# dselivanov/rsparse

Measured on AMD Instinct MI355X. Metric: als_iterations_per_sec, higher is better.
Workload: dtype f32 (Gram products of rows > 512 / <= 32 non-zeros as 2 x fp16 / 3 x bf16 split terms of the fp32 operands, fp32 accumulate; everything else fp32); 1 GPU; WRMF implicit ALS, CG(3), synthetic 10000000x1000000, 500155883 nnz, rank 128, lambda 0.1; survey_config=3, feedback=implicit, n_items=1000000, nnz=500155883, rank=128, solver=conjugate_gradient, cg_steps=3, parallelism=rows sharded x1, factors replicated

## Files before the change

rsparse_amd/csrc/wrmf_cg_mf.hip:

```cpp
#include <cstdio>
#include <utility>

#pragma clang diagnostic ignored "-Winline-asm"

#include "wrmf_internal.h"
#include "wrmf_device.h"

namespace rsparse_hip {
namespace {
using namespace dev;
constexpr int MF_A0 = 0;
#define MF_TOP "a255"
}
}

#include "wrmf_mf.h"

namespace rsparse_hip {
namespace {

constexpr float kCgTolMf = 1e-10f;
__device__ __forceinline__ void cgm_operands_hi(const float (&x)[16], f16x8& h0, f16x8& h1) {
  float b0[8], b1[8];
#pragma unroll
  for (int e = 0; e < 8; e++) {
    const auto sw2 = __builtin_amdgcn_permlane32_swap(__float_as_uint(x[e]), __float_as_uint(x[8 + e]), false, false);
    b0[e] = __uint_as_float(sw2[0]);
    b1[e] = __uint_as_float(sw2[1]);
  }
  unsigned hh0[4], hh1[4];
#pragma unroll
  for (int q = 0; q < 4; q++) {
    const f32x2 v0 = {b0[2 * q], b0[2 * q + 1]}, v1 = {b1[2 * q], b1[2 * q + 1]};
    hh0[q] = __builtin_bit_cast(unsigned, __builtin_convertvector(v0, f16x2));
    hh1[q] = __builtin_bit_cast(unsigned, __builtin_convertvector(v1, f16x2));
  }
  h0 = mf_pack(hh0[0], hh0[1], hh0[2], hh0[3]);
  h1 = mf_pack(hh1[0], hh1[1], hh1[2], hh1[3]);
}

struct CgmOps {
  f16x8 ah[4], al[4], mh[4];
};
struct CgmProd {
  int T, kind, K, I;
};
constexpr CgmProd cgm_prod(int idx) {
  if (idx < 16) return {mf_tid(idx % 4, 0), idx / 4, 0, idx % 4};
  idx -= 16;
  if (idx < 12) return {mf_tid(1 + idx % 3, 1), idx / 3, 1, 1 + idx % 3};
  idx -= 12;
  const int w = idx % 3, K = w == 2 ? 3 : 2, I = w == 0 ? 2 : 3;
  return {mf_tid(I, K), idx / 3, K, I};
}
template <int T>
__device__ __forceinline__ void cgm_mma16(const f16x8& a, const f16x8& b) {
  asm volatile("v_mfma_f32_32x32x16_f16 a[%c2:%c3], %0, %1, a[%c2:%c3]" ::"v"(a), "v"(b), "i"(MF_A0 + 16 * T), "i"(MF_A0 + 16 * T + 15));
}

template <int NOPS>
struct CgmWave {
  union {
    float ring[3][2048];
    float T[32 * 36];
  };
  int midx[3][64];
  float mval[3][64];
  float gval[3][64];
  unsigned long long maddr[3][64];
  float vec[128];
  float x0[128];
  float rhs[128];
  double loss;
};
template <int NOPS>
struct CgmSmem {
  float4 G[10][64][4];
  CgmWave<NOPS> w[4];
};

template <class RD, class GV, class WV>
__device__ __forceinline__ void cgm_matvec(RD&& rd, GV&& gtile, WV& sw, const int n, const int hf, const int ln,
                                           const float (&pr)[4], float (&out)[4]) {
  wave_sync();
  if (hf == 0) {
#pragma unroll
    for (int I = 0; I < 4; I++) sw.vec[32 * I + n] = pr[I];
  }
  wave_sync();
  float dsum[4] = {0.f, 0.f, 0.f, 0.f};
  mf_sfor<4>([&](auto kt) {
    constexpr int K = decltype(kt)::value;
    float pc[16];
#pragma unroll
    for (int q = 0; q < 4; q++) {
      const float4 t = *reinterpret_cast<const float4*>(&sw.vec[32 * K + 8 * q + 4 * hf]);
      pc[4 * q] = t.x; pc[4 * q + 1] = t.y; pc[4 * q + 2] = t.z; pc[4 * q + 3] = t.w;
    }
    float ts[16];
#pragma unroll
    for (int v = 0; v < 16; v++) ts[v] = 0.f;
    mf_sfor<4 - K>([&](auto st) {
      constexpr int I = K + decltype(st)::value;
      constexpr int T = mf_tid(I, K);
      float g[16];
      gtile(std::integral_constant<int, T>{}, g);
      mf_sfor<16>([&](auto vt) {
        constexpr int v = decltype(vt)::value;
        const float av = rd(std::integral_constant<int, T>{}, std::integral_constant<int, v>{}) + g[v];
        dsum[I] = fmaf(av, pc[v], dsum[I]);
        if constexpr (I > K) ts[v] = fmaf(av, pr[I], ts[v]);
// ... 152 lines not shown
              constexpr int I = K + decltype(st2)::value;
              constexpr int T = mf_tid(I, K);
              if constexpr (T < 6) mf_mma16<10 + T>(mh[K], mh[I]);
              else hi[T - 6] = __builtin_amdgcn_mfma_f32_32x32x16_f16(mh[K], mh[I], hi[T - 6], 0, 0, 0);
            });
          });
        };
        float gj;
        if constexpr (SYM) gj = inl ? __builtin_amdgcn_sqrtf(fmaxf(cvr - 1.f, 0.f) * sw_) : 0.f;
        else gj = f1;
        if constexpr (SYM) {
          cgm_operands_hi(xm0, mh[0], mh[1]);
          cgm_operands_hi(xm1, mh[2], mh[3]);
          __builtin_amdgcn_sched_barrier(0);
          m2_products();
          __builtin_amdgcn_sched_barrier(0);
        } else {
          mf_operands(xm0, bh[0], bl[0], bh[1], bl[1]);
          mf_operands(xm1, bh[2], bl[2], bh[3], bl[3]);
#pragma unroll
          for (int t = 0; t < 4; t++) mh[t] = bh[t];
          __builtin_amdgcn_sched_barrier(0);
          m2_products();
          __builtin_amdgcn_sched_barrier(0);
        }
#pragma unroll
        for (int s2 = 0; s2 < 16; s2++) {
          const float s_a = readlane_f(gj, s2);
          xs0[s2] *= s_a;
          xs1[s2] *= s_a;
        }
        mf_operands(xs0, ah[0], al[0], ah[1], al[1]);
        __builtin_amdgcn_sched_barrier(0);
        mf_operands(xs1, ah[2], al[2], ah[3], al[3]);
        __builtin_amdgcn_sched_barrier(0);
        mf_sfor<3>([&](auto pt) {
          constexpr int pr = decltype(pt)::value;
          mf_sfor<4>([&](auto kt) {
            constexpr int K = decltype(kt)::value;
            mf_sfor<4 - K>([&](auto st2) {
              constexpr int I = K + decltype(st2)::value;
              if constexpr (SYM) mf_mma16<mf_tid(I, K)>(pr == 2 ? al[K] : ah[K], pr == 1 ? al[I] : ah[I]);
              else mf_mma16<mf_tid(I, K)>(pr == 2 ? al[K] : ah[K], pr == 1 ? bl[I] : bh[I]);
            });
          });
        });
      };
      CgmOps OA, OB;
      if constexpr (SYM) {
        const f16x8 z = mf_pack(0u, 0u, 0u, 0u);
#pragma unroll
        for (int t = 0; t < 4; t++) { OA.ah[t] = z; OA.al[t] = z; OA.mh[t] = z; }
      }
      auto mm = [&](auto it, const CgmOps& P) __attribute__((always_inline)) {
        constexpr CgmProd pd = cgm_prod(decltype(it)::value);
        if constexpr (pd.kind == 0) {
          if constexpr (pd.T < 6) cgm_mma16<10 + pd.T>(P.mh[pd.K], P.mh[pd.I]);
          else hi[pd.T - 6] = __builtin_amdgcn_mfma_f32_32x32x16_f16(P.mh[pd.K], P.mh[pd.I], hi[pd.T - 6], 0, 0, 0);
        } else {
          cgm_mma16<pd.T>(pd.kind == 3 ? P.al[pd.K] : P.ah[pd.K], pd.kind == 2 ? P.al[pd.I] : P.ah[pd.I]);
        }
      };
      auto transform = [&](const int c) __attribute__((always_inline)) {
        const int cs = c % 3;
        int l2 = ln;
        asm volatile("" : "+v"(l2));
        const float cvr = sw.mval[cs][l2];
        const int id = sw.midx[cs][l2];
        if constexpr (SYM) csum += p1 + 64 * c + l2 < p2 ? cvr : 0.f;
        wave_sync();
        sw.maddr[cs][l2] = (unsigned long long)(unsigned)id * (k * 4) - (long long)(((l2 & 7) - 4) * 1024);
        if constexpr (SYM) sw.gval[cs][l2] = __builtin_amdgcn_sqrtf(fmaxf(cvr - 1.f, 0.f) * sw_);
        wave_sync();
      };
      auto zero_tail = [&](const int slot, const int ccnt) __attribute__((always_inline)) {
        float* rs = &sw.ring[slot][0];
#pragma unroll 1
        for (int jz = ccnt; jz < 16; jz++) {
          rs[(jz & 7) * 256 + (jz >> 3) * 128 + ln] = 0.f;
          rs[(jz & 7) * 256 + (jz >> 3) * 128 + 64 + ln] = 0.f;
        }
        wave_sync();
      };
      auto step_sym = [&](const int slot, const int cs, auto jt, const CgmOps& P, CgmOps& N, const float4 va0, const float4 vb0, const float2 wc0, const float2 wg0) __attribute__((always_inline)) {
        constexpr int j = decltype(jt)::value;
        const float* rs = &sw.ring[slot][0] + 128 * hfl + 4 * (ln & 31);
        const float2* pc = reinterpret_cast<const float2*>(&sw.mval[cs][16 * j + 8 * hfl]);
        const float2* pg = reinterpret_cast<const float2*>(&sw.gval[cs][16 * j + 8 * hfl]);
        float2 wc[2], wg[2];
        wc[0] = wc0;
        wg[0] = wg0;
        float4 va[2], vb[2];
        va[0] = va0;
        vb[0] = vb0;
        unsigned hm[4][4], hh[4][4], ll[4][4];
        mf_sfor<4>([&](auto qt) {
          constexpr int q = decltype(qt)::value;
          if constexpr (q < 3) {
            va[(q + 1) & 1] = *reinterpret_cast<const float4*>(rs + (2 * q + 2) * 256);
            vb[(q + 1) & 1] = *reinterpret_cast<const float4*>(rs + (2 * q + 3) * 256);
            wc[(q + 1) & 1] = pc[q + 1];
            wg[(q + 1) & 1] = pg[q + 1];
          }
          const float c0 = wc[q & 1].x, c1 = wc[q & 1].y, g0 = wg[q & 1].x, g1 = wg[q & 1].y;
          const float4 xa = va[q & 1], xb = vb[q & 1];
          const float a0s[4] = {xa.x, xa.y, xa.z, xa.w}, a1s[4] = {xb.x, xb.y, xb.z, xb.w};
          mf_sfor<4>([&](auto It) {
            constexpr int I = decltype(It)::value, u = 4 * q + I, m0 = (5 * u) / 2, m1 = (5 * (u + 1)) / 2;
            const float a0 = a0s[I], a1 = a1s[I];
            ua[I] = fmaf(c1, a1, fmaf(c0, a0, ua[I]));
            const float t0 = a0 * sx, t1 = a1 * sx;
            {
              const f32x2 tv = {t0, t1};
              hm[I][q] = __builtin_bit_cast(unsigned, __builtin_convertvector(tv, f16x2));
            }
            mm(std::integral_constant<int, m0>{}, P);
            __builtin_amdgcn_sched_barrier(0);
            {
              const f32x2 yv = {t0 * g0, t1 * g1};
              const unsigned hv = __builtin_bit_cast(unsigned, __builtin_convertvector(yv, f16x2));
              float r0, r1;
              asm("v_fma_mix_f32 %0, %1, %2, -%3 op_sel_hi:[0,0,1]" : "=v"(r0) : "v"(t0), "v"(g0), "v"(hv));
              asm("v_fma_mix_f32 %0, %1, %2, -%3 op_sel:[0,0,1] op_sel_hi:[0,0,1]" : "=v"(r1) : "v"(t1), "v"(g1), "v"(hv));
              const f32x2 rv = {r0, r1};
              hh[I][q] = hv;
              ll[I][q] = __builtin_bit_cast(unsigned, __builtin_convertvector(rv, f16x2));
            }
            mm(std::integral_constant<int, m0 + 1>{}, P);
            if constexpr (m1 - m0 == 3) {
              __builtin_amdgcn_sched_barrier(0);
              mm(std::integral_constant<int, m0 + 2>{}, P);
            }
            __builtin_amdgcn_sched_barrier(0);
          });
        });
#pragma unroll
        for (int I = 0; I < 4; I++) {
          N.mh[I] = mf_pack(hm[I][0], hm[I][1], hm[I][2], hm[I][3]);
          N.ah[I] = mf_pack(hh[I][0], hh[I][1], hh[I][2], hh[I][3]);
          N.al[I] = mf_pack(ll[I][0], ll[I][1], ll[I][2], ll[I][3]);
        }
      };
      wave_sync();
      request_meta(0);
      request_meta(1);
      asm volatile("s_waitcnt vmcnt(0)" ::: "memory");
      transform(0);
      request(0, 0);
      request(1, 1);
      const int tail_st = ((p2 - p1) & 15) ? nsteps - 1 : -1;
      int slot = 0;
      for (int c = 0; 4 * c < nsteps; c++) {
        bool done = false;
        mf_sfor<4>([&](auto jt) {
          constexpr int j = decltype(jt)::value;
          const int st = 4 * c + j;
          if (done || st >= nsteps) { done = true; return; }
          const int slot2 = slot == 0 ? 2 : slot - 1;
          float4 fva, fvb;
          float2 fwc, fwg;
          auto first_reads = [&](const int sl, const int cs, const int jj) __attribute__((always_inline)) {
            const float* rs = &sw.ring[sl][0] + 128 * hfl + 4 * (ln & 31);
            fva = *reinterpret_cast<const float4*>(rs);
            fvb = *reinterpret_cast<const float4*>(rs + 256);
            fwc = *reinterpret_cast<const float2*>(&sw.mval[cs][16 * jj + 8 * hfl]);
            fwg = *reinterpret_cast<const float2*>(&sw.gval[cs][16 * jj + 8 * hfl]);
          };
          if constexpr (j == 1) transform(c + 1);
          const bool more = st + 2 < nsteps;
          if (more) {
            if constexpr (j == 1) asm volatile("s_waitcnt vmcnt(10)" ::: "memory");
            else asm volatile("s_waitcnt vmcnt(8)" ::: "memory");
            if constexpr (SYM) first_reads(slot, c % 3, j);
            request(st + 2, slot2);
            if constexpr (j == 0) request_meta(c + 2);
          } else {
            asm volatile("s_waitcnt vmcnt(0)" ::: "memory");
            if constexpr (SYM) {
              if (st == tail_st) zero_tail(slot, (p2 - p1) & 15);
              first_reads(slot, c % 3, j);
            }
          }
          if constexpr (SYM) {
            __builtin_amdgcn_sched_barrier(0);
            if constexpr (j & 1) step_sym(slot, c % 3, jt, OB, OA, fva, fvb, fwc, fwg);
            else step_sym(slot, c % 3, jt, OA, OB, fva, fvb, fwc, fwg);
          } else {
            const float cvr = sw.mval[c % 3][16 * j + (ln & 15)];
            const float* rs = &sw.ring[slot][0];
            float xs0[16], xs1[16];
#pragma unroll
            for (int s2 = 0; s2 < 16; s2++) {
              xs0[s2] = rs[(s2 & 7) * 256 + (s2 >> 3) * 128 + 4 * (ln & 31) + hfl];
              xs1[s2] = rs[(s2 & 7) * 256 + (s2 >> 3) * 128 + 4 * (ln & 31) + 2 + hfl];
            }
            __builtin_amdgcn_sched_barrier(0);
            consume(st, cvr, xs0, xs1);
            __builtin_amdgcn_sched_barrier(0);
          }
          slot = slot == 2 ? 0 : slot + 1;
        });
        if (done) break;
      }
      if constexpr (SYM) {
        if (nsteps & 1) mf_sfor<40>([&](auto it) { mm(it, OB); });
        else mf_sfor<40>([&](auto it) { mm(it, OA); });
#pragma unroll
        for (int I = 0; I < 4; I++) {
          const unsigned du = __float_as_uint(ua[I]);
          const auto sw2 = __builtin_amdgcn_permlane32_swap(du, du, false, false);
          ua[I] = __uint_as_float(sw2[0]) + __uint_as_float(sw2[1]);
        }
      }
      wave_sync();
    }
    ln = lane;
    asm volatile("" : "+v"(ln));
    const int n = ln & 31, hf = ln >> 5;
    const float un_m1 = (un1 * un1) * (SYM ? unw : unw), un_m2 = un1 * un1;
    MF_DRAIN();
    mf_sfor<160>([&](auto rt) {
      constexpr int R = decltype(rt)::value;
      mf_wr<R>(mf_rd<R>() * un_m1);
    });
    mf_sfor<96>([&](auto rt) {
      constexpr int R = 160 + decltype(rt)::value;
      mf_wr<R>(mf_rd<R>() * un_m2);
    });
    {
      float um = un_m2;
      asm volatile("" : "+v"(um));
#pragma unroll
      for (int t = 0; t < 4; t++)
#pragma unroll
        for (int e = 0; e < 16; e++) hi[t][e] *= um;
    }
    float b[4], x[4];
    if constexpr (SYM) {
#pragma unroll
      for (int I = 0; I < 4; I++) {
        b[I] = ua[I];
        x[I] = sw.x0[4 * n + I];
      }
    } else {
      wave_sync();
      sw.rhs[ln] = u0;
      sw.rhs[64 + ln] = u1;
      wave_sync();
#pragma unroll
      for (int I = 0; I < 4; I++) {
        b[I] = sw.rhs[32 * I + n];
        x[I] = sw.x0[4 * n + I];
      }
    }
    auto rd_m1 = [&](auto tt, auto vt) { return mf_rd<16 * decltype(tt)::value + decltype(vt)::value>(); };
    auto g_tile = [&](auto tt, float (&g)[16]) {
      constexpr int T = decltype(tt)::value;
#pragma unroll
      for (int q = 0; q < 4; q++) {
        const float4 t = sm.G[T][ln][q];
        g[4 * q] = t.x; g[4 * q + 1] = t.y; g[4 * q + 2] = t.z; g[4 * q + 3] = t.w;
      }
    };
    float r[4], p[4], ap[4];
    cgm_matvec(rd_m1, g_tile, sw, n, hf, ln, x, ap);
#pragma unroll
    for (int I = 0; I < 4; I++) { r[I] = b[I] - ap[I]; p[I] = r[I]; }
    double rsold = (double)cgm_dot(r, r, hf);
    for (int stp = 0; stp < a.cg_steps; stp++) {
      cgm_matvec(rd_m1, g_tile, sw, n, hf, ln, p, ap);
      const float alpha = (float)(rsold / (double)cgm_dot(p, ap, hf));
#pragma unroll
      for (int I = 0; I < 4; I++) { x[I] = fmaf(alpha, p[I], x[I]); r[I] = fmaf(-alpha, ap[I], r[I]); }
// ... 92 lines not shown
```

rsparse_amd/csrc/wrmf_kernels.hip:

```cpp
#include "wrmf_internal.h"
#include "wrmf_device.h"

namespace rsparse_hip {
namespace {

using namespace dev;

constexpr float kCgTol = 1e-10f;

template <int KP, int T, int W, bool IMPLICIT>
struct CgSmem {
  static constexpr int LDT = Geo<KP>::LDT;
  static constexpr size_t gram_floats = IMPLICIT ? (size_t)KP * KP : 0;
  static constexpr size_t tile_floats = (size_t)W * T * LDT;
  static constexpr size_t vec_floats = (size_t)W * KP;
  static constexpr size_t red_floats = (size_t)2 * W * KP + 2 * W;
  static constexpr size_t short_bytes = (gram_floats + tile_floats + vec_floats) * 4 + 16;
  static constexpr size_t long_bytes = (gram_floats + tile_floats + vec_floats + red_floats) * 4 + 16;
};

template <int KP, int W>
__device__ __forceinline__ void load_gram_lds(float* sG, const float* __restrict__ G, int k, int tid) {
  for (int e = tid; e < KP * KP; e += W * 64) {
    const int r = e / KP, c = e % KP;
// ... 251 lines not shown
          for (int u = 0; u < EPL; u++) out[u] = fmaf(mode == 0 ? -lam_use : lam_use, v[u], out[u]);
        } else if (gb && mode == 0) {
#pragma unroll
          for (int u = 0; u < EPL; u++) out[u] += (active && e0 + u < k) ? a.rhs_init[e0 + u] : 0.f;
        }
      }
      buf ^= 1;
    };

    float dummy = 0.f;
    sweep(x, 0, r, dummy);
    float rs = 0.f;
#pragma unroll
    for (int u = 0; u < EPL; u++) { p[u] = r[u]; rs = fmaf(r[u], r[u], rs); }
    float rsold = wave_sum(rs);
    for (int it = 0; it < a.cg_steps; ++it) {
      sweep(p, 1, ap, dummy);
      float pap = 0.f;
#pragma unroll
      for (int u = 0; u < EPL; u++) pap = fmaf(p[u], ap[u], pap);
      pap = wave_sum(pap);
      const float alpha = (float)((double)rsold / (double)pap);
      rs = 0.f;
#pragma unroll
      for (int u = 0; u < EPL; u++) {
        x[u] = fmaf(alpha, p[u], x[u]);
        r[u] = fmaf(-alpha, ap[u], r[u]);
        rs = fmaf(r[u], r[u], rs);
      }
      const float rsnew = wave_sum(rs);
      if (rsnew < kCgTol) break;
      const float beta = (float)((double)rsnew / (double)rsold);
#pragma unroll
      for (int u = 0; u < EPL; u++) p[u] = fmaf(p[u], beta, r[u]);
      rsold = rsnew;
    }
    float rl = 0.f;
    sweep(x, 2, ap, rl);
    float xx = 0.f;
#pragma unroll
    for (int u = 0; u < EPL; u++) xx = fmaf(x[u], x[u], xx);
    xx = wave_sum(xx);
    if (wv == 0) {
      wloss += IMPLICIT ? (double)rl + a.lambda_loss * (double)xx : (double)(rl + lam_use * xx);
#pragma unroll
      for (int u = 0; u < EPL; u++)
        if (active && e0 + u < k) yrow[e0 + u] = x[u];
    }
  }
  if (tid == 0) a.loss_partials[loss_slot0 + blockIdx.x] = wloss;
}

typedef float f32x16 __attribute__((ext_vector_type(16)));

template <int KP>
__global__ __launch_bounds__(256, 2) void gramian_partial_kernel(const float* __restrict__ X, int k, int64_t n,
                                                              float* __restrict__ partials,
                                                              unsigned* __restrict__ absmax_bits) {
  constexpr int NT = KP / 32, U = 4;
  const int lane = threadIdx.x & 63;
  const int64_t gw = (int64_t)blockIdx.x * 4 + (threadIdx.x >> 6), nw = (int64_t)gridDim.x * 4;
  const int col = lane & 31, half = lane >> 5;
  f32x16 acc[NT][NT];
#pragma unroll
  for (int i = 0; i < NT; i++)
#pragma unroll
    for (int j = 0; j < NT; j++)
#pragma unroll
      for (int e = 0; e < 16; e++) acc[i][j][e] = 0.f;

  float amax = 0.f;
  auto fetch = [&](const int64_t n0, float (&dst)[U][NT]) {
#pragma unroll
    for (int u = 0; u < U; u++) {
      const int64_t ent = n0 + 2 * u + half;
      const int64_t er = ent < n ? ent : n - 1;
#pragma unroll
      for (int mt = 0; mt < NT; mt++) dst[u][mt] = X[er * k + min(mt * 32 + col, k - 1)];
    }
  };
  auto take = [&](const int64_t n0, const float (&src)[U][NT], float (&dst)[U][NT]) {
#pragma unroll
    for (int u = 0; u < U; u++) {
      const bool in = n0 + 2 * u + half < n;
#pragma unroll
      for (int mt = 0; mt < NT; mt++) dst[u][mt] = src[u][mt] * ((in && mt * 32 + col < k) ? 1.f : 0.f);
    }
  };
  float av[U][NT], nx[U][NT];
  const int64_t stride = nw * 2 * U;
  int64_t n0 = gw * 2 * U;
  if (n0 < n) {
    fetch(n0, nx);
    take(n0, nx, av);
  }
  for (; n0 < n; n0 += stride) {
    const bool more = n0 + stride < n;
    if (more) fetch(n0 + stride, nx);
#pragma unroll
    for (int u = 0; u < U; u++)
#pragma unroll
      for (int mt = 0; mt < NT; mt++) amax = fmaxf(amax, fabsf(av[u][mt]));
#pragma unroll
    for (int u = 0; u < U; u++)
#pragma unroll
      for (int mt = 0; mt < NT; mt++)
#pragma unroll
        for (int nt = 0; nt <= mt; nt++)
          acc[mt][nt] = __builtin_amdgcn_mfma_f32_32x32x2f32(av[u][mt], av[u][nt], acc[mt][nt], 0, 0, 0);
    if (more) take(n0 + stride, nx, av);
  }
  if (absmax_bits) {
#pragma unroll
    for (int off = 32; off > 0; off >>= 1) amax = fmaxf(amax, __shfl_xor(amax, off));
    if (lane == 0) atomicMax(absmax_bits, __float_as_uint(amax < 3.0e38f ? amax : 3.0e38f));
  }
  float* out = partials + (size_t)gw * KP * KP;
#pragma unroll
  for (int mt = 0; mt < NT; mt++)
#pragma unroll
    for (int nt = 0; nt <= mt; nt++)
#pragma unroll
      for (int e = 0; e < 16; e++) {
        const int rr = mt * 32 + (e & 3) + 8 * (e >> 2) + 4 * half;
        out[(size_t)rr * KP + nt * 32 + col] = acc[mt][nt][e];
      }
}

__global__ void gramian_reduce_kernel(const float* __restrict__ partials, int nparts, int KP, int k, float ridge,
                                      float* __restrict__ G, double* __restrict__ diag) {
  const int e = blockIdx.x * blockDim.x + threadIdx.x;
  if (e >= k * k) return;
  const int aa = e / k, bb = e % k;
  const int ta = aa / 32, tb = bb / 32;
  const int rr = ta >= tb ? aa : bb, cc = ta >= tb ? bb : aa;
  double s = 0.0;
  const float* src = partials + (size_t)rr * KP + cc;
  for (int w = 0; w < nparts; w++) s += (double)src[(size_t)w * KP * KP];
  G[(size_t)bb * k + aa] = (float)s + (aa == bb ? ridge : 0.f);
  if (aa == bb) diag[aa] = s;
}

__global__ void trace_kernel(const double* __restrict__ diag, int k, double* __restrict__ out) {
  if (threadIdx.x == 0 && blockIdx.x == 0) {
    double s = 0.0;
    for (int i = 0; i < k; i++) s += diag[i];
    *out = s;
  }
}

__global__ __launch_bounds__(256) void weighted_sumsq_kernel(const float* __restrict__ X, int k, int64_t n,
                                                             const float* __restrict__ w, double* __restrict__ partials) {
  __shared__ double sh[4];
  const int64_t total = n * k;
  double s = 0.0;
  for (int64_t e = (int64_t)blockIdx.x * 256 + threadIdx.x; e < total; e += (int64_t)gridDim.x * 256) {
    const float v = X[e];
    const float wj = w ? w[e / k] : 1.f;
    s += (double)(v * v * wj);
  }
  for (int m = 32; m >= 1; m >>= 1) s += __shfl_xor(s, m);
  if ((threadIdx.x & 63) == 0) sh[threadIdx.x >> 6] = s;
  __syncthreads();
  if (threadIdx.x == 0) partials[blockIdx.x] = (sh[0] + sh[1]) + (sh[2] + sh[3]);
}

__global__ __launch_bounds__(256) void sum_partials_kernel(const double* __restrict__ partials, size_t n,
                                                           double* __restrict__ out) {
  __shared__ double sh[4];
  double s = 0.0;
  for (size_t e = threadIdx.x; e < n; e += 256) s += partials[e];
  for (int m = 32; m >= 1; m >>= 1) s += __shfl_xor(s, m);
  if ((threadIdx.x & 63) == 0) sh[threadIdx.x >> 6] = s;
  __syncthreads();
  if (threadIdx.x == 0) *out = (sh[0] + sh[1]) + (sh[2] + sh[3]);
}

__global__ __launch_bounds__(256) void sum_partials_stage_kernel(const double* __restrict__ partials, size_t n,
                                                                 double* __restrict__ tail) {
  __shared__ double sh[4];
  const size_t per = (n + gridDim.x - 1) / gridDim.x, lo = (size_t)blockIdx.x * per, hi = lo + per < n ? lo + per : n;
  double s = 0.0;
  for (size_t e = lo + threadIdx.x; e < hi; e += 256) s += partials[e];
  for (int m = 32; m >= 1; m >>= 1) s += __shfl_xor(s, m);
  if ((threadIdx.x & 63) == 0) sh[threadIdx.x >> 6] = s;
  __syncthreads();
  if (threadIdx.x == 0) tail[blockIdx.x] = (sh[0] + sh[1]) + (sh[2] + sh[3]);
}

__global__ void f64_to_f32_kernel(const double* __restrict__ in, float* __restrict__ out, size_t n) {
  for (size_t e = (size_t)blockIdx.x * blockDim.x + threadIdx.x; e < n; e += (size_t)gridDim.x * blockDim.x)
    out[e] = (float)in[e];
}
__global__ void f32_to_f64_kernel(const float* __restrict__ in, double* __restrict__ out, size_t n) {
  for (size_t e = (size_t)blockIdx.x * blockDim.x + threadIdx.x; e < n; e += (size_t)gridDim.x * blockDim.x)
    out[e] = (double)in[e];
}

template <typename K>
hipError_t set_lds(K kernel, size_t bytes) {
// ... 25 lines not shown
    if ((err = hipGetLastError()) != hipSuccess) return err;
  }
  if (ev && (err = hipEventRecord(ev[2], s)) != hipSuccess) return err;
  return hipSuccess;
}

}

int padded_rank(int k) {
  if (k <= 0) return 0;
  if (k <= 32) return 32;
  if (k <= 64) return 64;
  if (k <= 128) return 128;
  return 0;
}

size_t cg_loss_slots(int n_cols, int n_long) {
  const size_t grid_s = ((size_t)n_cols + kRowsPerWGShort - 1) / kRowsPerWGShort;
  const size_t grid_l = ((size_t)n_long + kRowsPerWGLong - 1) / kRowsPerWGLong;
  return grid_s * kWavesPerWG + grid_l;
}

size_t chol_loss_slots(int n_cols) {
  return (size_t)(n_cols < kCholMaxGrid ? (n_cols > 0 ? n_cols : 1) : kCholMaxGrid);
}

hipError_t launch_als_cg(const AlsArgs& a, bool implicit, hipStream_t s, hipEvent_t* ev) {
  const int KP = padded_rank(a.k);
  const bool vec = (a.k % 4 == 0) && ((reinterpret_cast<uintptr_t>(a.X) & 15) == 0);
#define RSP_DISPATCH(KPV)                                                             \
  if (KP == KPV) {                                                                    \
    if (implicit) return vec ? launch_cg_t<KPV, true, true>(a, s, ev) : launch_cg_t<KPV, true, false>(a, s, ev); \
    return vec ? launch_cg_t<KPV, false, true>(a, s, ev) : launch_cg_t<KPV, false, false>(a, s, ev);             \
  }
  RSP_DISPATCH(32)
  RSP_DISPATCH(64)
  RSP_DISPATCH(128)
#undef RSP_DISPATCH
  return hipErrorInvalidValue;
}

hipError_t launch_sum_partials(const double* partials, size_t n, double* out, hipStream_t s, double* tail) {
  if (tail && n > 16384) {
    hipLaunchKernelGGL(sum_partials_stage_kernel, dim3(kSumStageBlocks), dim3(256), 0, s, partials, n, tail);
    hipError_t err = hipGetLastError();
    if (err != hipSuccess) return err;
    hipLaunchKernelGGL(sum_partials_kernel, dim3(1), dim3(256), 0, s, tail, (size_t)kSumStageBlocks, out);
    return hipGetLastError();
  }
  hipLaunchKernelGGL(sum_partials_kernel, dim3(1), dim3(256), 0, s, partials, n, out);
  return hipGetLastError();
}

static int gramian_waves(int64_t n) {
  int64_t w = (n + 63) / 64;
  if (w < 1) w = 1;
  if (w > 1024) w = 1024;
  return (int)((w + 3) / 4 * 4);
}

size_t gramian_scratch_floats(int k, int64_t n) {
  const int KP = padded_rank(k);
  return (size_t)gramian_waves(n) * KP * KP + 2 * 128  + 16;
}

hipError_t launch_gramian(const float* X, int k, int64_t n, float ridge, float* XtX, double* sumsq,
                          float* scratch, hipStream_t s, hipEvent_t* ev, unsigned* absmax_bits) {
  const int KP = padded_rank(k);
  if (!KP) return hipErrorInvalidValue;
  const int waves = gramian_waves(n);
  float* partials = scratch;
  double* diag = reinterpret_cast<double*>(scratch + (((size_t)waves * KP * KP + 1) & ~(size_t)1));
  const int grid = waves / 4;
  if (ev) (void)hipEventRecord(ev[0], s);
  prof_note(ev, KP == 32 ? reinterpret_cast<const void*>(gramian_partial_kernel<32>)
                         : (KP == 64 ? reinterpret_cast<const void*>(gramian_partial_kernel<64>)
                                     : reinterpret_cast<const void*>(gramian_partial_kernel<128>)));
  prof_note(ev ? ev + 1 : nullptr, reinterpret_cast<const void*>(gramian_reduce_kernel));
  if (KP == 32) hipLaunchKernelGGL(gramian_partial_kernel<32>, dim3(grid), dim3(256), 0, s, X, k, n, partials, absmax_bits);
  else if (KP == 64) hipLaunchKernelGGL(gramian_partial_kernel<64>, dim3(grid), dim3(256), 0, s, X, k, n, partials, absmax_bits);
  else hipLaunchKernelGGL(gramian_partial_kernel<128>, dim3(grid), dim3(256), 0, s, X, k, n, partials, absmax_bits);
  hipError_t err = hipGetLastError();
  if (err != hipSuccess) return err;
  if (ev) (void)hipEventRecord(ev[1], s);
  hipLaunchKernelGGL(gramian_reduce_kernel, dim3((k * k + 255) / 256), dim3(256), 0, s, partials, waves, KP, k,
                     ridge, XtX, diag);
  if ((err = hipGetLastError()) != hipSuccess) return err;
  if (sumsq) {
    hipLaunchKernelGGL(trace_kernel, dim3(1), dim3(64), 0, s, diag, k, sumsq);
    err = hipGetLastError();
  }
  if (ev) (void)hipEventRecord(ev[2], s);
  return err;
}

hipError_t launch_weighted_sumsq(const float* X, int k, int64_t n, const float* w, double* out, double* scratch,
                                 hipStream_t s) {
  int64_t blocks = (n * k + 256 * 16 - 1) / (256 * 16);
  if (blocks < 1) blocks = 1;
  if (blocks > 1024) blocks = 1024;
  hipLaunchKernelGGL(weighted_sumsq_kernel, dim3((int)blocks), dim3(256), 0, s, X, k, n, w, scratch);
  hipError_t err = hipGetLastError();
  if (err != hipSuccess) return err;
  return launch_sum_partials(scratch, (size_t)blocks, out, s);
}

hipError_t launch_f64_to_f32(const double* in, float* out, size_t n, hipStream_t s) {
  if (!n) return hipSuccess;
  size_t blocks = (n + 1023) / 1024;
  if (blocks > 4096) blocks = 4096;
  hipLaunchKernelGGL(f64_to_f32_kernel, dim3((int)blocks), dim3(256), 0, s, in, out, n);
  return hipGetLastError();
}
hipError_t launch_f32_to_f64(const float* in, double* out, size_t n, hipStream_t s) {
  if (!n) return hipSuccess;
  size_t blocks = (n + 1023) / 1024;
  if (blocks > 4096) blocks = 4096;
  hipLaunchKernelGGL(f32_to_f64_kernel, dim3((int)blocks), dim3(256), 0, s, in, out, n);
  return hipGetLastError();
}

}
```

Measured before the change: 8.506 iterations/s.

## Merge symmetric cross terms of split-fp16 Gram into doubled products

Reorders the split-precision product schedule for the symmetric Gram case. On diagonal tiles the hi*lo and lo*hi cross terms are merged into one MFMA against a doubled low operand, which cuts the per-row products from 40 to 36. Afterwards each diagonal 32x32 accumulator tile is symmetrized through LDS (averaged with its transpose) to restore exact symmetry. This adds VALU doubling work, LDS round trips in the epilogue, and a small precision risk from doubling the fp16 low part.

```diff
diff --git a/rsparse_amd/csrc/wrmf_cg_mf.hip b/rsparse_amd/csrc/wrmf_cg_mf.hip
--- a/rsparse_amd/csrc/wrmf_cg_mf.hip
+++ b/rsparse_amd/csrc/wrmf_cg_mf.hip
@@ -45,18 +45,38 @@
 struct CgmProd {
   int T, kind, K, I;
 };
+constexpr int kCgmProds = 36;
 constexpr CgmProd cgm_prod(int idx) {
-  if (idx < 16) return {mf_tid(idx % 4, 0), idx / 4, 0, idx % 4};
-  idx -= 16;
-  if (idx < 12) return {mf_tid(1 + idx % 3, 1), idx / 3, 1, 1 + idx % 3};
-  idx -= 12;
-  const int w = idx % 3, K = w == 2 ? 3 : 2, I = w == 0 ? 2 : 3;
-  return {mf_tid(I, K), idx / 3, K, I};
-}
+  constexpr int tab[kCgmProds][3] = {
+      {0, 0, 0}, {0, 0, 1}, {0, 0, 2}, {0, 0, 3}, {1, 0, 0}, {1, 0, 1}, {1, 0, 2}, {1, 0, 3}, {2, 0, 0}, {2, 0, 1}, {2, 0, 2}, {2, 0, 3},
+      {3, 0, 1}, {3, 0, 2}, {3, 0, 3},
+      {0, 1, 1}, {0, 1, 2}, {2, 1, 1}, {0, 1, 3}, {1, 1, 1}, {1, 1, 2}, {1, 1, 3}, {2, 1, 2}, {2, 1, 3}, {3, 1, 2}, {3, 1, 3},
+      {2, 2, 2}, {0, 2, 2}, {0, 2, 3}, {0, 3, 3}, {1, 2, 3}, {1, 2, 2}, {2, 2, 3}, {1, 3, 3}, {3, 2, 3}, {2, 3, 3}};
+  return {mf_tid(tab[idx][2], tab[idx][1]), tab[idx][0], tab[idx][1], tab[idx][2]};
+}
+constexpr bool cgm_doubled(int idx) { return cgm_prod(idx).kind == 2 && cgm_prod(idx).I == cgm_prod(idx).K; }
+constexpr int cgm_doubled_in(int m0, int m1) {
+  for (int i = m0; i < m1; i++)
+    if (cgm_doubled(i)) return i;
+  return -1;
+}
+constexpr bool cgm_table_ok() {
+  int seen[10][4] = {};
+  for (int i = 0; i < kCgmProds; i++) {
+    const CgmProd p = cgm_prod(i);
+    if (p.I < p.K || p.I > 3 || p.kind > 3 || (p.kind == 3 && p.I == p.K)) return false;
+    if (seen[p.T][p.kind]++) return false;
+    if (i && cgm_prod(i - 1).T == p.T && (cgm_prod(i - 1).kind == 0) == (p.kind == 0)) return false;
+    if (cgm_doubled(i) != (i == 8 || i == 17 || i == 26 || i == 35)) return false;
+  }
+  return true;
+}
+static_assert(cgm_table_ok(), "cgm_prod");
 template <int T>
 __device__ __forceinline__ void cgm_mma16(const f16x8& a, const f16x8& b) {
   asm volatile("v_mfma_f32_32x32x16_f16 a[%c2:%c3], %0, %1, a[%c2:%c3]" ::"v"(a), "v"(b), "i"(MF_A0 + 16 * T), "i"(MF_A0 + 16 * T + 15));
 }
+__device__ __forceinline__ f16x8 cgm_twice(const f16x8& l) { return l + l; }
 
 template <int NOPS>
 struct CgmWave {
@@ -315,11 +335,13 @@
 #pragma unroll
         for (int t = 0; t < 4; t++) { OA.ah[t] = z; OA.al[t] = z; OA.mh[t] = z; }
       }
-      auto mm = [&](auto it, const CgmOps& P) __attribute__((always_inline)) {
+      auto mm = [&](auto it, const CgmOps& P, const f16x8& b2) __attribute__((always_inline)) {
         constexpr CgmProd pd = cgm_prod(decltype(it)::value);
         if constexpr (pd.kind == 0) {
           if constexpr (pd.T < 6) cgm_mma16<10 + pd.T>(P.mh[pd.K], P.mh[pd.I]);
           else hi[pd.T - 6] = __builtin_amdgcn_mfma_f32_32x32x16_f16(P.mh[pd.K], P.mh[pd.I], hi[pd.T - 6], 0, 0, 0);
+        } else if constexpr (cgm_doubled(decltype(it)::value)) {
+          cgm_mma16<pd.T>(P.ah[pd.K], b2);
         } else {
           cgm_mma16<pd.T>(pd.kind == 3 ? P.al[pd.K] : P.ah[pd.K], pd.kind == 2 ? P.al[pd.I] : P.ah[pd.I]);
         }
@@ -369,15 +391,22 @@
           const float4 xa = va[q & 1], xb = vb[q & 1];
           const float a0s[4] = {xa.x, xa.y, xa.z, xa.w}, a1s[4] = {xb.x, xb.y, xb.z, xb.w};
           mf_sfor<4>([&](auto It) {
-            constexpr int I = decltype(It)::value, u = 4 * q + I, m0 = (5 * u) / 2, m1 = (5 * (u + 1)) / 2;
+            constexpr int I = decltype(It)::value, u = 4 * q + I, m0 = (9 * u) / 4, m1 = (9 * (u + 1)) / 4;
             const float a0 = a0s[I], a1 = a1s[I];
+            constexpr int md = cgm_doubled_in(m0, m1);
+            f16x8 b2 = P.al[0];
+            if constexpr (md >= 0) b2 = cgm_twice(P.al[cgm_prod(md >= 0 ? md : 0).I]);
             ua[I] = fmaf(c1, a1, fmaf(c0, a0, ua[I]));
             const float t0 = a0 * sx, t1 = a1 * sx;
             {
               const f32x2 tv = {t0, t1};
               hm[I][q] = __builtin_bit_cast(unsigned, __builtin_convertvector(tv, f16x2));
             }
-            mm(std::integral_constant<int, m0>{}, P);
+            if constexpr (md >= 0) {
+              static_assert(md < 0 || md == m0 + 2, "the copy's distance to its matrix instruction");
+              asm volatile("" : "+v"(b2));
+            }
+            mm(std::integral_constant<int, m0>{}, P, b2);
             __builtin_amdgcn_sched_barrier(0);
             {
               const f32x2 yv = {t0 * g0, t1 * g1};
@@ -389,10 +418,10 @@
               hh[I][q] = hv;
               ll[I][q] = __builtin_bit_cast(unsigned, __builtin_convertvector(rv, f16x2));
             }
-            mm(std::integral_constant<int, m0 + 1>{}, P);
+            mm(std::integral_constant<int, m0 + 1>{}, P, b2);
             if constexpr (m1 - m0 == 3) {
               __builtin_amdgcn_sched_barrier(0);
-              mm(std::integral_constant<int, m0 + 2>{}, P);
+              mm(std::integral_constant<int, m0 + 2>{}, P, b2);
             }
             __builtin_amdgcn_sched_barrier(0);
           });
@@ -466,8 +495,15 @@
         if (done) break;
       }
       if constexpr (SYM) {
-        if (nsteps & 1) mf_sfor<40>([&](auto it) { mm(it, OB); });
-        else mf_sfor<40>([&](auto it) { mm(it, OA); });
+        auto last_mm = [&](const CgmOps& P) __attribute__((always_inline)) {
+          f16x8 b2[4];
+#pragma unroll
+          for (int I = 0; I < 4; I++) b2[I] = cgm_twice(P.al[I]);
+          asm volatile("s_nop 1" : "+v"(b2[0]), "+v"(b2[1]), "+v"(b2[2]), "+v"(b2[3]));
+          mf_sfor<kCgmProds>([&](auto it) { mm(it, P, b2[cgm_prod(decltype(it)::value).I]); });
+        };
+        if (nsteps & 1) last_mm(OB);
+        else last_mm(OA);
 #pragma unroll
         for (int I = 0; I < 4; I++) {
           const unsigned du = __float_as_uint(ua[I]);
@@ -482,6 +518,23 @@
     const int n = ln & 31, hf = ln >> 5;
     const float un_m1 = (un1 * un1) * (SYM ? unw : unw), un_m2 = un1 * un1;
     MF_DRAIN();
+    if constexpr (SYM) {
+      mf_sfor<4>([&](auto dt) {
+        constexpr int R0 = 16 * mf_tid(decltype(dt)::value, decltype(dt)::value);
+        float d[16];
+        mf_sfor<16>([&](auto vt) { d[decltype(vt)::value] = mf_rd<R0 + decltype(vt)::value>(); });
+        wave_sync();
+#pragma unroll
+        for (int q = 0; q < 4; q++)
+          *reinterpret_cast<float4*>(&sw.T[n * 36 + 8 * q + 4 * hf]) = make_float4(d[4 * q], d[4 * q + 1], d[4 * q + 2], d[4 * q + 3]);
+        wave_sync();
+        mf_sfor<16>([&](auto vt) {
+          constexpr int v = decltype(vt)::value;
+          mf_wr<R0 + v>(0.5f * (d[v] + sw.T[(8 * (v >> 2) + 4 * hf + (v & 3)) * 36 + n]));
+        });
+      });
+      wave_sync();
+    }
     mf_sfor<160>([&](auto rt) {
       constexpr int R = decltype(rt)::value;
       mf_wr<R>(mf_rd<R>() * un_m1);
```

After: 8.547 iterations/s (median of 6 runs). No clear change (+0.5%).

## Rewrite Gramian with 3-term bf16 split MFMA, LDS partial sums, fused reduce

Applied to the files above, without the earlier changes.

Replaces the fp32 32x32x2 MFMA Gramian with a bf16 32x32x16 MFMA path. Each fp32 operand is split into three bf16 terms and six cross-products are accumulated. Rows are fetched with buffer loads in a prefetching chain, and an exponent lift guards tiny inputs. Per-wave accumulators are flushed into LDS and summed per workgroup, which cuts the partial count from up to 1024 waves to 256 workgroups. The reduce kernel now reads float4 partials, writes both triangles of G, and folds the trace into a last-block-done atomic, which drops a kernel launch. Risks include precision loss from the bf16 split, heavy register and LDS pressure at occupancy 1, and a changed lane-to-column mapping that must match the reduce indexing.

```diff
diff --git a/rsparse_amd/csrc/wrmf_kernels.hip b/rsparse_amd/csrc/wrmf_kernels.hip
--- a/rsparse_amd/csrc/wrmf_kernels.hip
+++ b/rsparse_amd/csrc/wrmf_kernels.hip
@@ -327,100 +327,247 @@
 }
 
 typedef float f32x16 __attribute__((ext_vector_type(16)));
-
-template <int KP>
-__global__ __launch_bounds__(256, 2) void gramian_partial_kernel(const float* __restrict__ X, int k, int64_t n,
+typedef float f32x2g __attribute__((ext_vector_type(2)));
+typedef __bf16 bf16x2g __attribute__((ext_vector_type(2)));
+typedef __bf16 bf16x8g __attribute__((ext_vector_type(8)));
+typedef unsigned u32x4g __attribute__((ext_vector_type(4)));
+
+constexpr int kGramTrip = 16;
+constexpr int kGramMaxWGs = 256;
+constexpr int kGramChain = 4;
+
+__host__ __device__ constexpr int gram_tiles(int KP) { return (KP / 32) * (KP / 32 + 1) / 2; }
+__host__ __device__ constexpr int gram_partial_floats(int KP) { return gram_tiles(KP) * 16 * 64; }
+
+__device__ __forceinline__ unsigned gram_split_stage(f32x2g& r, bool last) {
+  const bf16x2g hb = __builtin_convertvector(r, bf16x2g);
+  const unsigned pk = __builtin_bit_cast(unsigned, hb);
+  if (!last) {
+    const f32x2g hi = {__uint_as_float(pk << 16), __uint_as_float(pk & 0xffff0000u)};
+    r -= hi;
+  }
+  return pk;
+}
+__device__ __forceinline__ f32x16 gram_mfma(const u32x4g a, const u32x4g b, const f32x16 c) {
+  return __builtin_amdgcn_mfma_f32_32x32x16_bf16(__builtin_bit_cast(bf16x8g, a), __builtin_bit_cast(bf16x8g, b), c, 0, 0,
+                                                 0);
+}
+
+template <int KP, bool VEC>
+__global__ __launch_bounds__(256, 1) void gramian_partial_kernel(const float* __restrict__ X, int k, int64_t n,
                                                               float* __restrict__ partials,
-                                                              unsigned* __restrict__ absmax_bits) {
-  constexpr int NT = KP / 32, U = 4;
-  const int lane = threadIdx.x & 63;
-  const int64_t gw = (int64_t)blockIdx.x * 4 + (threadIdx.x >> 6), nw = (int64_t)gridDim.x * 4;
-  const int col = lane & 31, half = lane >> 5;
+                                                              unsigned* __restrict__ absmax_bits,
+                                                              unsigned* __restrict__ done_count) {
+  constexpr int NT = KP / 32, E = kGramTrip / 2;
+  typedef float rowv __attribute__((ext_vector_type(NT)));
+  constexpr int TILES = gram_tiles(KP);
+  extern __shared__ __attribute__((aligned(16))) float gsum[];
+  const int lane = threadIdx.x & 63, wv = rfl(threadIdx.x >> 6);
+  const int64_t gw = (int64_t)blockIdx.x * 4 + wv, nw = (int64_t)gridDim.x * 4;
+  const int row = lane & 31, half = lane >> 5;
+  if (done_count && blockIdx.x == 0 && threadIdx.x == 0) *done_count = 0;
   f32x16 acc[NT][NT];
-#pragma unroll
-  for (int i = 0; i < NT; i++)
-#pragma unroll
-    for (int j = 0; j < NT; j++)
-#pragma unroll
-      for (int e = 0; e < 16; e++) acc[i][j][e] = 0.f;
+  float4* mysum = reinterpret_cast<float4*>(gsum + wv * TILES * 1024) + lane;
+
+  bool cin[NT];
+#pragma unroll
+  for (int I = 0; I < NT; I++) cin[I] = NT * row + I < k;
 
   float amax = 0.f;
-  auto fetch = [&](const int64_t n0, float (&dst)[U][NT]) {
-#pragma unroll
-    for (int u = 0; u < U; u++) {
-      const int64_t ent = n0 + 2 * u + half;
-      const int64_t er = ent < n ? ent : n - 1;
-#pragma unroll
-      for (int mt = 0; mt < NT; mt++) dst[u][mt] = X[er * k + min(mt * 32 + col, k - 1)];
+  float rawA[E][NT], rawB[E][NT];
+  unsigned voff[VEC ? 1 : NT];
+#pragma unroll
+  for (int I = 0; I < (VEC ? 1 : NT); I++)
+    voff[I] = (unsigned)(E * half * k + (VEC ? min(NT * row, k - NT) : min(NT * row + I, k - 1))) * 4u;
+  auto fetch = [&](float (&raw)[E][NT], const int64_t n0) {
+    const int rem = (int)max((int64_t)0, min((int64_t)kGramTrip, n - n0));
+#pragma unroll
+    for (int j = 0; j < E; j++) {
+      const __amdgpu_buffer_rsrc_t rs = __builtin_amdgcn_make_buffer_rsrc(
+          const_cast<float*>(X + (n0 + j) * k), 0, j < rem ? (rem - j) * k * 4 : 0, 0x00020000);
+      if constexpr (VEC && NT == 4) {
+        const u32x4g v = __builtin_amdgcn_raw_buffer_load_b128(rs, voff[0], 0, 0);
+#pragma unroll
+        for (int I = 0; I < NT; I++) raw[j][I] = __uint_as_float(v[I]);
+      } else if constexpr (VEC && NT == 2) {
+        typedef unsigned u32x2g __attribute__((ext_vector_type(2)));
+        const u32x2g v = __builtin_amdgcn_raw_buffer_load_b64(rs, voff[0], 0, 0);
+        raw[j][0] = __uint_as_float(v[0]);
+        raw[j][1] = __uint_as_float(v[1]);
+      } else {
+#pragma unroll
+        for (int I = 0; I < NT; I++)
+          raw[j][I] = __uint_as_float(__builtin_amdgcn_raw_buffer_load_b32(rs, voff[VEC ? 0 : I], 0, 0));
+      }
     }
   };
-  auto take = [&](const int64_t n0, const float (&src)[U][NT], float (&dst)[U][NT]) {
-#pragma unroll
-    for (int u = 0; u < U; u++) {
-      const bool in = n0 + 2 * u + half < n;
-#pragma unroll
-      for (int mt = 0; mt < NT; mt++) dst[u][mt] = src[u][mt] * ((in && mt * 32 + col < k) ? 1.f : 0.f);
-    }
+  const int64_t stride = nw * kGramTrip;
+  int lift = -1;
+  float lift_f = 1.f;
+  auto trip = [&](float (&raw)[E][NT], const int64_t n_next) {
+    __builtin_amdgcn_sched_barrier(0);
+    u32x4g term[NT][3];
+#pragma unroll
+    for (int j = 0; j < E; j += 2)
+#pragma unroll
+      for (int I = 0; I < NT; I++) {
+        f32x2g r = {cin[I] ? raw[j][I] * lift_f : 0.f, cin[I] ? raw[j + 1][I] * lift_f : 0.f};
+        amax = fmaxf(amax, fmaxf(fabsf(r.x), fabsf(r.y)));
+        term[I][0][j / 2] = gram_split_stage(r, false);
+        term[I][1][j / 2] = gram_split_stage(r, false);
+        term[I][2][j / 2] = gram_split_stage(r, true);
+      }
+    __builtin_amdgcn_sched_barrier(0);
+    fetch(raw, n_next);
+    __builtin_amdgcn_sched_barrier(0);
+#pragma unroll
+    for (int mt = 0; mt < NT; mt++)
+#pragma unroll
+      for (int nt = 0; nt <= mt; nt++) {
+        f32x16 c = acc[mt][nt];
+        c = gram_mfma(term[mt][0], term[nt][0], c);
+        c = gram_mfma(term[mt][0], term[nt][1], c);
+        c = gram_mfma(term[mt][1], term[nt][0], c);
+        c = gram_mfma(term[mt][0], term[nt][2], c);
+        c = gram_mfma(term[mt][2], term[nt][0], c);
+        c = gram_mfma(term[mt][1], term[nt][1], c);
+        acc[mt][nt] = c;
+      }
   };
-  float av[U][NT], nx[U][NT];
-  const int64_t stride = nw * 2 * U;
-  int64_t n0 = gw * 2 * U;
-  if (n0 < n) {
-    fetch(n0, nx);
-    take(n0, nx, av);
-  }
-  for (; n0 < n; n0 += stride) {
-    const bool more = n0 + stride < n;
-    if (more) fetch(n0 + stride, nx);
-#pragma unroll
-    for (int u = 0; u < U; u++)
-#pragma unroll
-      for (int mt = 0; mt < NT; mt++) amax = fmaxf(amax, fabsf(av[u][mt]));
-#pragma unroll
-    for (int u = 0; u < U; u++)
+  for (;;) {
+#pragma unroll
+    for (int i = 0; i < NT; i++)
+#pragma unroll
+      for (int j = 0; j < NT; j++)
+#pragma unroll
+        for (int e = 0; e < 16; e++) acc[i][j][e] = 0.f;
+    for (int i = 0; i < TILES * 4; i++) mysum[i * 64] = make_float4(0.f, 0.f, 0.f, 0.f);
+    amax = 0.f;
+    int64_t n0 = gw * kGramTrip;
+    fetch(rawA, n0);
+    fetch(rawB, n0 + stride);
+    if (lift < 0) {
+      float m = 0.f;
+#pragma unroll
+      for (int j = 0; j < E; j++)
+#pragma unroll
+        for (int I = 0; I < NT; I++) m = fmaxf(m, cin[I] ? fabsf(rawA[j][I]) : 0.f);
+#pragma unroll
+      for (int off = 32; off > 0; off >>= 1) m = fmaxf(m, __shfl_xor(m, off));
+      lift = (m > 0.f && m < 0x1p-40f) ? rfl(-40 - ilogbf(m)) : 0;
+      lift_f = ldexpf(1.f, lift);
+    }
+    for (; n0 < n; n0 += kGramChain * stride) {
+      trip(rawA, n0 + 2 * stride);
+      if (n0 + stride < n) trip(rawB, n0 + 3 * stride);
+      if (n0 + 2 * stride < n) trip(rawA, n0 + 4 * stride);
+      if (n0 + 3 * stride < n) trip(rawB, n0 + 5 * stride);
+      int t = 0;
 #pragma unroll
       for (int mt = 0; mt < NT; mt++)
 #pragma unroll
-        for (int nt = 0; nt <= mt; nt++)
-          acc[mt][nt] = __builtin_amdgcn_mfma_f32_32x32x2f32(av[u][mt], av[u][nt], acc[mt][nt], 0, 0, 0);
-    if (more) take(n0 + stride, nx, av);
+        for (int nt = 0; nt <= mt; nt++, t++)
+#pragma unroll
+          for (int e = 0; e < 16; e += 4) {
+            float4 v = mysum[(t * 4 + e / 4) * 64];
+            v.x += acc[mt][nt][e];
+            v.y += acc[mt][nt][e + 1];
+            v.z += acc[mt][nt][e + 2];
+            v.w += acc[mt][nt][e + 3];
+            mysum[(t * 4 + e / 4) * 64] = v;
+            acc[mt][nt][e] = acc[mt][nt][e + 1] = acc[mt][nt][e + 2] = acc[mt][nt][e + 3] = 0.f;
+          }
+    }
+#pragma unroll
+    for (int off = 32; off > 0; off >>= 1) amax = fmaxf(amax, __shfl_xor(amax, off));
+    if (lift == 0 || amax <= 0x1p30f) break;
+    lift = 0;
+    lift_f = 1.f;
+  }
+  if (lift) {
+    amax = ldexpf(amax, -lift);
+    for (int i = 0; i < TILES * 4; i++) {
+      float4 v = mysum[i * 64];
+      v.x = ldexpf(v.x, -2 * lift);
+      v.y = ldexpf(v.y, -2 * lift);
+      v.z = ldexpf(v.z, -2 * lift);
+      v.w = ldexpf(v.w, -2 * lift);
+      mysum[i * 64] = v;
+    }
   }
   if (absmax_bits) {
-#pragma unroll
-    for (int off = 32; off > 0; off >>= 1) amax = fmaxf(amax, __shfl_xor(amax, off));
     if (lane == 0) atomicMax(absmax_bits, __float_as_uint(amax < 3.0e38f ? amax : 3.0e38f));
   }
-  float* out = partials + (size_t)gw * KP * KP;
-#pragma unroll
-  for (int mt = 0; mt < NT; mt++)
-#pragma unroll
-    for (int nt = 0; nt <= mt; nt++)
-#pragma unroll
-      for (int e = 0; e < 16; e++) {
-        const int rr = mt * 32 + (e & 3) + 8 * (e >> 2) + 4 * half;
-        out[(size_t)rr * KP + nt * 32 + col] = acc[mt][nt][e];
-      }
-}
-
-__global__ void gramian_reduce_kernel(const float* __restrict__ partials, int nparts, int KP, int k, float ridge,
-                                      float* __restrict__ G, double* __restrict__ diag) {
-  const int e = blockIdx.x * blockDim.x + threadIdx.x;
-  if (e >= k * k) return;
-  const int aa = e / k, bb = e % k;
-  const int ta = aa / 32, tb = bb / 32;
-  const int rr = ta >= tb ? aa : bb, cc = ta >= tb ? bb : aa;
-  double s = 0.0;
-  const float* src = partials + (size_t)rr * KP + cc;
-  for (int w = 0; w < nparts; w++) s += (double)src[(size_t)w * KP * KP];
-  G[(size_t)bb * k + aa] = (float)s + (aa == bb ? ridge : 0.f);
-  if (aa == bb) diag[aa] = s;
-}
-
-__global__ void trace_kernel(const double* __restrict__ diag, int k, double* __restrict__ out) {
-  if (threadIdx.x == 0 && blockIdx.x == 0) {
-    double s = 0.0;
-    for (int i = 0; i < k; i++) s += diag[i];
-    *out = s;
+  __syncthreads();
+  float* out = partials + (size_t)blockIdx.x * gram_partial_floats(KP);
+  for (int t = 0; t < TILES; t++) {
+    const int i = (t * 4 + wv) * 256 + lane * 4;
+    const float4 a0 = *reinterpret_cast<const float4*>(gsum + i), a1 = *reinterpret_cast<const float4*>(gsum + TILES * 1024 + i);
+    const float4 a2 = *reinterpret_cast<const float4*>(gsum + 2 * TILES * 1024 + i);
+    const float4 a3 = *reinterpret_cast<const float4*>(gsum + 3 * TILES * 1024 + i);
+    const float r[4] = {(a0.x + a1.x) + (a2.x + a3.x), (a0.y + a1.y) + (a2.y + a3.y), (a0.z + a1.z) + (a2.z + a3.z),
+                        (a0.w + a1.w) + (a2.w + a3.w)};
+#pragma unroll
+    for (int q = 0; q < 4; q++) out[(t * 16 + 4 * wv + q) * 64 + lane] = r[q];
+  }
+}
+
+__global__ __launch_bounds__(256) void gramian_reduce_kernel(const float* __restrict__ partials, int nparts, int KP, int k,
+                                                             float ridge, float* __restrict__ G, double* diag,
+                                                             unsigned* done_count, double* __restrict__ sumsq) {
+  __shared__ double sh[16][64];
+  __shared__ bool last;
+  const int tid = threadIdx.x, q = tid & 15, g = tid >> 4;
+  const int NT = KP / 32;
+  const size_t pf = (size_t)gram_partial_floats(KP);
+  const float* src = partials + (size_t)blockIdx.x * 64 + 4 * q;
+  double s0 = 0.0, s1 = 0.0, s2 = 0.0, s3 = 0.0;
+#pragma unroll 4
+  for (int p = g; p < nparts; p += 16) {
+    const float4 v = *reinterpret_cast<const float4*>(src + p * pf);
+    s0 += (double)v.x;
+    s1 += (double)v.y;
+    s2 += (double)v.z;
+    s3 += (double)v.w;
+  }
+  sh[g][4 * q + 0] = s0;
+  sh[g][4 * q + 1] = s1;
+  sh[g][4 * q + 2] = s2;
+  sh[g][4 * q + 3] = s3;
+  __syncthreads();
+  for (int h = 8; h >= 1; h >>= 1) {
+    if (g < h)
+#pragma unroll
+      for (int u = 0; u < 4; u++) sh[g][4 * q + u] += sh[g + h][4 * q + u];
+    __syncthreads();
+  }
+  if (tid < 64) {
+    const int t = blockIdx.x / 16, e = blockIdx.x % 16;
+    int mt = 0;
+    while ((mt + 1) * (mt + 2) / 2 <= t) mt++;
+    const int nt = t - mt * (mt + 1) / 2;
+    const int i = (e & 3) + 8 * (e >> 2) + 4 * (tid >> 5), j = tid & 31;
+    const int a = NT * i + mt, b = NT * j + nt;
+    const double s = sh[0][tid];
+    if (a < k && b < k && (mt != nt || i >= j)) {
+      const float v = (float)s + (a == b ? ridge : 0.f);
+      G[(size_t)a * k + b] = v;
+      G[(size_t)b * k + a] = v;
+      if (a == b && sumsq) diag[a] = s;
+    }
+  }
+  if (!sumsq) return;
+  __threadfence();
+  __syncthreads();
+  if (tid == 0) last = atomicAdd(done_count, 1u) == gridDim.x - 1;
+  __syncthreads();
+  if (last && tid < 64) {
+    __threadfence();
+    double v = 0.0;
+    if (tid < k) v = __hip_atomic_load(diag + tid, __ATOMIC_RELAXED, __HIP_MEMORY_SCOPE_AGENT);
+    if (tid + 64 < k) v += __hip_atomic_load(diag + tid + 64, __ATOMIC_RELAXED, __HIP_MEMORY_SCOPE_AGENT);
+    for (int m = 32; m >= 1; m >>= 1) v += __shfl_xor(v, m);
+    if (tid == 0) *sumsq = v;
   }
 }
 
@@ -552,44 +699,50 @@
   return hipGetLastError();
 }
 
-static int gramian_waves(int64_t n) {
-  int64_t w = (n + 63) / 64;
+static int gramian_wgs(int64_t n) {
+  int64_t w = (n + 4 * kGramTrip - 1) / (4 * kGramTrip);
   if (w < 1) w = 1;
-  if (w > 1024) w = 1024;
-  return (int)((w + 3) / 4 * 4);
+  if (w > kGramMaxWGs) w = kGramMaxWGs;
+  return (int)w;
 }
 
 size_t gramian_scratch_floats(int k, int64_t n) {
   const int KP = padded_rank(k);
-  return (size_t)gramian_waves(n) * KP * KP + 2 * 128  + 16;
+  return (size_t)gramian_wgs(n) * gram_partial_floats(KP) + 2 * 128  + 16 ;
+}
+
+template <int KP>
+static hipError_t launch_gramian_partial(bool vec, int grid, hipStream_t s, hipEvent_t* ev, const float* X, int k, int64_t n,
+                                   float* partials, unsigned* absmax_bits, unsigned* done_count) {
+  auto kern = vec ? gramian_partial_kernel<KP, true> : gramian_partial_kernel<KP, false>;
+  const size_t lds = (size_t)4 * gram_partial_floats(KP) * sizeof(float);
+  hipError_t err = set_lds(kern, lds);
+  if (err != hipSuccess) return err;
+  prof_note(ev, reinterpret_cast<const void*>(kern));
+  hipLaunchKernelGGL(kern, dim3(grid), dim3(256), lds, s, X, k, n, partials, absmax_bits, done_count);
+  return hipGetLastError();
 }
 
 hipError_t launch_gramian(const float* X, int k, int64_t n, float ridge, float* XtX, double* sumsq,
                           float* scratch, hipStream_t s, hipEvent_t* ev, unsigned* absmax_bits) {
   const int KP = padded_rank(k);
   if (!KP) return hipErrorInvalidValue;
-  const int waves = gramian_waves(n);
+  const int grid = gramian_wgs(n), NT = KP / 32;
   float* partials = scratch;
-  double* diag = reinterpret_cast<double*>(scratch + (((size_t)waves * KP * KP + 1) & ~(size_t)1));
-  const int grid = waves / 4;
+  double* diag = reinterpret_cast<double*>(scratch + (size_t)grid * gram_partial_floats(KP));
+  unsigned* done_count = reinterpret_cast<unsigned*>(diag + 128);
+  const bool vec = (k % NT == 0) && ((reinterpret_cast<uintptr_t>(X) & (size_t)(4 * NT - 1)) == 0);
   if (ev) (void)hipEventRecord(ev[0], s);
-  prof_note(ev, KP == 32 ? reinterpret_cast<const void*>(gramian_partial_kernel<32>)
-                         : (KP == 64 ? reinterpret_cast<const void*>(gramian_partial_kernel<64>)
-                                     : reinterpret_cast<const void*>(gramian_partial_kernel<128>)));
+  hipError_t err;
+  if (KP == 32) err = launch_gramian_partial<32>(vec, grid, s, ev, X, k, n, partials, absmax_bits, done_count);
+  else if (KP == 64) err = launch_gramian_partial<64>(vec, grid, s, ev, X, k, n, partials, absmax_bits, done_count);
+  else err = launch_gramian_partial<128>(vec, grid, s, ev, X, k, n, partials, absmax_bits, done_count);
+  if (err != hipSuccess) return err;
   prof_note(ev ? ev + 1 : nullptr, reinterpret_cast<const void*>(gramian_reduce_kernel));
-  if (KP == 32) hipLaunchKernelGGL(gramian_partial_kernel<32>, dim3(grid), dim3(256), 0, s, X, k, n, partials, absmax_bits);
-  else if (KP == 64) hipLaunchKernelGGL(gramian_partial_kernel<64>, dim3(grid), dim3(256), 0, s, X, k, n, partials, absmax_bits);
-  else hipLaunchKernelGGL(gramian_partial_kernel<128>, dim3(grid), dim3(256), 0, s, X, k, n, partials, absmax_bits);
-  hipError_t err = hipGetLastError();
-  if (err != hipSuccess) return err;
   if (ev) (void)hipEventRecord(ev[1], s);
-  hipLaunchKernelGGL(gramian_reduce_kernel, dim3((k * k + 255) / 256), dim3(256), 0, s, partials, waves, KP, k,
-                     ridge, XtX, diag);
-  if ((err = hipGetLastError()) != hipSuccess) return err;
-  if (sumsq) {
-    hipLaunchKernelGGL(trace_kernel, dim3(1), dim3(64), 0, s, diag, k, sumsq);
-    err = hipGetLastError();
-  }
+  hipLaunchKernelGGL(gramian_reduce_kernel, dim3(gram_partial_floats(KP) / 64), dim3(256), 0, s, partials, grid, KP, k,
+                     ridge, XtX, diag, done_count, sumsq);
+  err = hipGetLastError();
   if (ev) (void)hipEventRecord(ev[2], s);
   return err;
 }
```

Measured after the change: 8.502 iterations/s before, 8.536 iterations/s after, median of 6. Within noise of the previous version (+0.4%).
